# KerkDovan/univer-ocr

Measured on AMD Instinct MI355X. Metric: document-images/sec (fwd+bwd) on 256x512 synthetic pages, higher is better.
Workload: dtype f32; 1 GPU; BASELINE configs[2]: my_model train step (fwd+loss+bwd+L2+SGD) of Monochrome+Paragraph+Line on (32,256,512,1) pages and Char on (32,32,64,1) line strips per GPU; batch_per_gpu=32, global_batch=32, optimizer=sgd, parallelism=dp1, h2d_inclusive=False, input_grads=True, hip_graphs=True, pipelined_lanes=True, hw_queues=4

## Files before the change

### univer-ocr_amd/csrc/conv_fast.hip

```cpp
#include "finish_group.h"
#include "conv_dims.h"

namespace {

template <int C, typename TA>
__device__ __forceinline__ void load_vec(const TA* __restrict__ p, float (&v)[C]) {
    if constexpr (C == 1) {
        v[0] = ld1(p);
    } else if constexpr (C == 2) {
        const float2 t = ld2(p);
        v[0] = t.x;
        v[1] = t.y;
    } else {
        static_assert(C % 4 == 0, "channel count must be 1, 2 or a multiple of 4");
#pragma unroll
        for (int q = 0; q < C / 4; ++q) {
            const float4 t = ld4(p + 4 * q);
            v[4 * q] = t.x;
            v[4 * q + 1] = t.y;
            v[4 * q + 2] = t.z;
            v[4 * q + 3] = t.w;
        }
    }
}
// ... 179 lines not shown
        const bool row_ok = gy >= 0 && gy < d.oh;
        const int gyc = min(max(gy, 0), d.oh - 1);
#pragma unroll
        for (int c = 0; c < 3; ++c) {
            const int gx = i - 1 + c;
            load_vec<COUT>(gb + ((size_t)gyc * d.ow + min(max(gx, 0), d.ow - 1)) * COUT, g[r][c]);
            if (!(row_ok && gx >= 0 && gx < d.ow)) {
#pragma unroll
                for (int o = 0; o < COUT; ++o) g[r][c][o] = 0.f;
            }
        }
    }
    float out[2][2][CIN];
#pragma unroll
    for (int q = 0; q < 4; ++q)
#pragma unroll
        for (int ci = 0; ci < CIN; ++ci) out[q >> 1][q & 1][ci] = 0.f;
#pragma unroll
    for (int ky = 0; ky < 5; ++ky)
#pragma unroll
        for (int kx = 0; kx < 5; ++kx) {
            const int py = ky & 1, px = kx & 1;
            const int r = (py ? (3 - ky) / 2 : 1 - ky / 2) + 1, c = (px ? (3 - kx) / 2 : 1 - kx / 2) + 1;
#pragma unroll
            for (int ci = 0; ci < CIN; ++ci)
#pragma unroll
                for (int o = 0; o < COUT; ++o)
                    out[py][px][ci] += g[r][c][o] * w[((ky * 5 + kx) * CIN + ci) * COUT + o];
        }
#pragma unroll
    for (int py = 0; py < 2; ++py) {
        const int y = 2 * j + py;
        if (y >= d.h) break;
        const size_t off = (((size_t)b * d.h + y) * d.w + 2 * i) * CIN;
        if (CIN == 1 && (d.w & 1) == 0) {
            float v[2] = {out[py][0][0], out[py][1][0]};
            apply_mask<2>(v, mask_y, off, mask_act, mask_alpha);
            store_vec<2>(dx + off, v);
        } else {
#pragma unroll
            for (int px = 0; px < 2; ++px) {
                if (2 * i + px >= d.w) break;
                apply_mask<CIN>(out[py][px], mask_y, off + px * CIN, mask_act, mask_alpha);
                store_vec<CIN>(dx + off + px * CIN, out[py][px]);
            }
        }
    }
}

__global__ __launch_bounds__(256) void conv_dgrad_c64s2(const float* __restrict__ dy, const float* __restrict__ w,
                                                        float* __restrict__ dx, int n, int h, int wd, int oh, int ow,
                                                        const float* __restrict__ mask_y, int mask_act,
                                                        float mask_alpha) {
    constexpr int KH = 5, KW = 3, CO = 64;
    const int q = threadIdx.x & 15;
    const int b = blockIdx.z, y = blockIdx.y;
    const bool live = (int)(blockIdx.x * 16 + (threadIdx.x >> 4)) < wd;
    const int x = live ? blockIdx.x * 16 + (threadIdx.x >> 4) : wd - 1;
    const size_t pix = ((size_t)b * h + y) * wd + x;
    const float* gb = dy + (size_t)b * oh * ow * CO + 4 * q;
    float acc = 0.f;
#pragma unroll
    for (int t = 0; t < 3; ++t) {
        const int ky = (y & 1) + 2 * t, gy = (y - ky) / 2;
        if (ky >= KH || y - ky < 0 || gy >= oh) continue;
#pragma unroll
        for (int kx = 0; kx < KW; ++kx) {
            const int gx = x + 1 - kx;
            if (gx < 0 || gx >= ow) continue;
            const float4 g = *reinterpret_cast<const float4*>(gb + ((size_t)gy * ow + gx) * CO);
            const float4 wv = *reinterpret_cast<const float4*>(w + (ky * KW + kx) * CO + 4 * q);
            acc += g.x * wv.x + g.y * wv.y + g.z * wv.z + g.w * wv.w;
        }
    }
    acc += __shfl_xor(acc, 8, 64);
    acc += __shfl_xor(acc, 4, 64);
    acc += __shfl_xor(acc, 2, 64);
    acc += __shfl_xor(acc, 1, 64);
    if (!live || q != 0) return;
    if (mask_act != UOCR_ACT_NONE) acc *= act_grad_from_output<float>(mask_y[pix], mask_act, mask_alpha);
    dx[pix] = acc;
}

template <int N, int OFFS, typename TA>
__device__ __forceinline__ void load_row_c1(const TA* __restrict__ row, int a4, int width, bool row_ok,
                                            float fill, float (&seg)[N][1]) {
    constexpr int NV4 = (OFFS + N + 3) / 4;
    float buf[NV4 * 4];
#pragma unroll
    for (int k = 0; k < NV4; ++k) {
        const int col = a4 + 4 * k;
        float4 v = ld4(row + min(max(col, 0), width - 4));
        if (!(row_ok && col >= 0 && col < width)) v = make_float4(fill, fill, fill, fill);
        buf[4 * k] = v.x;
        buf[4 * k + 1] = v.y;
        buf[4 * k + 2] = v.z;
        buf[4 * k + 3] = v.w;
    }
#pragma unroll
    for (int j = 0; j < N; ++j) seg[j][0] = buf[OFFS + j];
}

template <int KH, int KW, int CIN, int COUT, int SH, int SW, int PX, typename TA, class K>
__global__ __launch_bounds__(256) void conv_fwd_px(const TA* __restrict__ x, const float* __restrict__ w,
                                                   const float* __restrict__ bias, TA* __restrict__ y,
                                                   FastDims d, float pad, int use_bias, int act, float alpha) {
    act = act_kind<K::act>(act);
    constexpr int NXV = (PX - 1) * SW + KW;
    const int ox0 = (blockIdx.x * 64 + threadIdx.x) * PX;
    const int oy = blockIdx.y * 4 + threadIdx.y;
    const int b = blockIdx.z;
    if (ox0 >= d.ow || oy >= d.oh) return;
    float acc[PX][COUT];
#pragma unroll
    for (int p = 0; p < PX; ++p)
#pragma unroll
        for (int o = 0; o < COUT; ++o) acc[p][o] = 0.f;
    const int ix0 = ox0 * SW - d.pw;
    const TA* xb = x + (size_t)b * d.h * d.w * CIN;
#pragma unroll 1
    for (int ky = 0; ky < KH; ++ky) {
        const int iy = oy * SH - d.ph + ky;
        const bool row_ok = iy >= 0 && iy < d.h;
        const TA* xr = xb + (size_t)min(max(iy, 0), d.h - 1) * d.w * CIN;
        const float* wr = w + ky * (KW * CIN * COUT);
        float xv[NXV][CIN];
        bool vec_done = false;
        if constexpr (CIN == 1 && PX % 4 == 0) {
            constexpr int PWC = KW / 2, OFFS = (4 - PWC % 4) % 4;
            if (d.pw == PWC && d.w % 4 == 0) {
                load_row_c1<NXV, OFFS>(xr, ix0 - OFFS, d.w, row_ok, pad, xv);
                vec_done = true;
            }
        }
        if (!vec_done) {
#pragma unroll
            for (int j = 0; j < NXV; ++j) {
                const int ix = ix0 + j;
                load_vec<CIN>(xr + (size_t)min(max(ix, 0), d.w - 1) * CIN, xv[j]);
                if (!(row_ok && ix >= 0 && ix < d.w)) {
#pragma unroll
                    for (int c = 0; c < CIN; ++c) xv[j][c] = pad;
                }
            }
        }
#pragma unroll
        for (int kx = 0; kx < KW; ++kx)
#pragma unroll
            for (int c = 0; c < CIN; ++c)
#pragma unroll
                for (int o = 0; o < COUT; ++o) {
                    const float wv = wr[(kx * CIN + c) * COUT + o];
#pragma unroll
                    for (int p = 0; p < PX; ++p) acc[p][o] += xv[p * SW + kx][c] * wv;
                }
    }
    if constexpr (COUT == 1 && PX % 4 == 0) {
        if (d.ow % PX == 0) {
            float out[PX];
#pragma unroll
            for (int p = 0; p < PX; ++p) out[p] = act_apply(acc[p][0] + (use_bias ? bias[0] : 0.f), act, alpha);
            store_vec<PX>(y + ((size_t)b * d.oh + oy) * d.ow + ox0, out);
            return;
        }
    }
#pragma unroll
    for (int p = 0; p < PX; ++p) {
        if (ox0 + p >= d.ow) break;
        float out[COUT];
#pragma unroll
        for (int o = 0; o < COUT; ++o) {
            float v = acc[p][o];
            if (use_bias) v += bias[o];
            out[o] = act_apply(v, act, alpha);
        }
        store_vec<COUT>(y + (((size_t)b * d.oh + oy) * d.ow + ox0 + p) * COUT, out);
    }
}

template <int KH, int KW, int CIN, int COUT, int PX, typename TA>
__global__ __launch_bounds__(256) void conv_dgrad_px(const TA* __restrict__ dy, const float* __restrict__ w,
                                                     TA* __restrict__ dx, FastDims d,
                                                     const TA* __restrict__ mask_y, int mask_act, float mask_alpha) {
    constexpr int NG = PX + KW - 1;
    const int ix0 = (blockIdx.x * 64 + threadIdx.x) * PX;
    const int iy = blockIdx.y * 4 + threadIdx.y;
    const int b = blockIdx.z;
    if (ix0 >= d.w || iy >= d.h) return;
    float acc[PX][CIN];
#pragma unroll
    for (int p = 0; p < PX; ++p)
#pragma unroll
        for (int c = 0; c < CIN; ++c) acc[p][c] = 0.f;
    const TA* gb = dy + (size_t)b * d.oh * d.ow * COUT;
    const int gx0 = ix0 + d.pw - (KW - 1);
#pragma unroll 1
    for (int ky = KH - 1; ky >= 0; --ky) {
        const int gy = iy + d.ph - ky;
        const bool row_ok = gy >= 0 && gy < d.oh;
        const TA* gr = gb + (size_t)min(max(gy, 0), d.oh - 1) * d.ow * COUT;
        const float* wr = w + ky * (KW * CIN * COUT);
        float g[NG][COUT];
        bool vec_done = false;
        if constexpr (COUT == 1 && PX % 4 == 0) {
            constexpr int PWC = KW / 2, OFFS = (((KW - 1 - PWC) % 4) + 4) % 4;
            if (d.pw == PWC && d.ow % 4 == 0) {
                load_row_c1<NG, OFFS>(gr, gx0 - OFFS, d.ow, row_ok, 0.f, g);
                vec_done = true;
            }
        }
        if (!vec_done) {
#pragma unroll
            for (int j = 0; j < NG; ++j) {
                const int gx = gx0 + j;
                load_vec<COUT>(gr + (size_t)min(max(gx, 0), d.ow - 1) * COUT, g[j]);
                if (!(row_ok && gx >= 0 && gx < d.ow)) {
#pragma unroll
                    for (int o = 0; o < COUT; ++o) g[j][o] = 0.f;
                }
            }
        }
#pragma unroll
        for (int kx = 0; kx < KW; ++kx)
#pragma unroll
            for (int c = 0; c < CIN; ++c)
#pragma unroll
                for (int o = 0; o < COUT; ++o) {
                    const float wv = wr[(kx * CIN + c) * COUT + o];
#pragma unroll
                    for (int p = 0; p < PX; ++p) acc[p][c] += g[p + (KW - 1) - kx][o] * wv;
                }
    }
    if constexpr (CIN == 1 && PX % 4 == 0) {
        if (d.w % PX == 0) {
            float out[PX];
#pragma unroll
            for (int p = 0; p < PX; ++p) out[p] = acc[p][0];
            const size_t off = ((size_t)b * d.h + iy) * d.w + ix0;
            apply_mask<PX>(out, mask_y, off, mask_act, mask_alpha);
            store_vec<PX>(dx + off, out);
            return;
        }
    }
#pragma unroll
    for (int p = 0; p < PX; ++p) {
        if (ix0 + p >= d.w) break;
        const size_t off = (((size_t)b * d.h + iy) * d.w + ix0 + p) * CIN;
        apply_mask<CIN>(acc[p], mask_y, off, mask_act, mask_alpha);
        store_vec<CIN>(dx + off, acc[p]);
    }
}

template <int KH, int KW, int PY, bool FLIP>
__global__ __launch_bounds__(256) void conv_c16_reduce(const float* __restrict__ src, const float* __restrict__ w,
                                                       const float* __restrict__ bias, float* __restrict__ dst,
                                                       int n, int h, int wd, int ph, int pw, float pad, int use_bias,
                                                       int act, float alpha, const float* __restrict__ mask_y,
                                                       int mask_act, float mask_alpha) {
    constexpr int C = 16, ROWS = PY + KH - 1;
    const int q = threadIdx.x & 3;
    const int ox = blockIdx.x * 16 + (threadIdx.x >> 2);
    const int oy0 = (blockIdx.y * 4 + threadIdx.y) * PY;
    const int b = blockIdx.z;
    float wreg[KH][KW][4];
#pragma unroll
    for (int ky = 0; ky < KH; ++ky)
#pragma unroll
        for (int kx = 0; kx < KW; ++kx) {
            const int sky = FLIP ? KH - 1 - ky : ky, skx = FLIP ? KW - 1 - kx : kx;
            const float4 t = *reinterpret_cast<const float4*>(w + (sky * KW + skx) * C + q * 4);
            wreg[ky][kx][0] = t.x;
            wreg[ky][kx][1] = t.y;
            wreg[ky][kx][2] = t.z;
            wreg[ky][kx][3] = t.w;
        }
    const int PH = FLIP ? KH - 1 - ph : ph, PW = FLIP ? KW - 1 - pw : pw;
    float acc[PY];
#pragma unroll
    for (int p = 0; p < PY; ++p) acc[p] = 0.f;
    const float* sb = src + (size_t)b * h * wd * C + q * 4;
    const int oxc = min(ox, wd - 1);
#pragma unroll
    for (int r = 0; r < ROWS; ++r) {
        const int iy = oy0 - PH + r;
        const bool row_ok = iy >= 0 && iy < h;
        const float* sr = sb + (size_t)min(max(iy, 0), h - 1) * wd * C;
#pragma unroll
        for (int kx = 0; kx < KW; ++kx) {
            const int ix = oxc - PW + kx;
            float4 v = *reinterpret_cast<const float4*>(sr + (size_t)min(max(ix, 0), wd - 1) * C);
            if (!(row_ok && ix >= 0 && ix < wd)) v = make_float4(pad, pad, pad, pad);
#pragma unroll
            for (int p = 0; p < PY; ++p) {
                const int ky = r - p;
                if (ky >= 0 && ky < KH)
                    acc[p] += v.x * wreg[ky][kx][0] + v.y * wreg[ky][kx][1] + v.z * wreg[ky][kx][2] +
                              v.w * wreg[ky][kx][3];
            }
        }
    }
#pragma unroll
    for (int p = 0; p < PY; ++p) {
        float v = acc[p];
        v += __shfl_xor(v, 1, 64);
        v += __shfl_xor(v, 2, 64);
        if (q == 0 && ox < wd && oy0 + p < h) {
            if (use_bias) v += bias[0];
            const size_t off = ((size_t)b * h + oy0 + p) * wd + ox;
            v = act_apply(v, act, alpha);
            if (mask_act != UOCR_ACT_NONE) v *= act_grad_from_output<float>(mask_y[off], mask_act, mask_alpha);
            dst[off] = v;
        }
    }
}
// ... 111 lines not shown
#pragma unroll
        for (int kx = 0; kx < KW; ++kx)
#pragma unroll
            for (int j = 0; j < 4; ++j) {
                float t = acc[ky][kx][j];
#pragma unroll
                for (int m = 4; m < 64; m <<= 1) t += __shfl_xor(t, m, 64);
                acc[ky][kx][j] = t;
            }
#pragma unroll
    for (int m = 4; m < 64; m <<= 1) accb += __shfl_xor(accb, m, 64);
    if (pl == 0) {
#pragma unroll
        for (int ky = 0; ky < KH; ++ky)
#pragma unroll
            for (int kx = 0; kx < KW; ++kx)
#pragma unroll
                for (int j = 0; j < 4; ++j) red[wv][q][(ky * KW + kx) * 4 + j] = acc[ky][kx][j];
        red[wv][q][NA - 1] = accb;
    }
    __syncthreads();
    const int tid = wv * 64 + threadIdx.x;
    float* out = partial + (size_t)blockIdx.x * 4 * NA;
    for (int a = tid; a < 4 * NA; a += 256) {
        const int qq = a / NA, i = a % NA;
        out[a] = red[0][qq][i] + red[1][qq][i] + red[2][qq][i] + red[3][qq][i];
    }
}

template <int KH, int KW>
__global__ __launch_bounds__(256) void conv_c16_wgrad_finish(const float* __restrict__ partial, float* __restrict__ dw,
                                                             float* __restrict__ db, int nblocks, int use_bias,
                                                             int accumulate) {
    constexpr int NA = KH * KW * 4 + 1;
    __shared__ double smem[16];
    const int i = blockIdx.x, q = blockIdx.y;
    double s = 0.0;
    for (int blk = threadIdx.x; blk < nblocks; blk += blockDim.x) s += (double)partial[((size_t)blk * 4 + q) * NA + i];
    s = block_reduce_sum(s, smem);
    if (threadIdx.x != 0) return;
    float* dst;
    if (i < NA - 1) {
        dst = dw + (i / 4) * 16 + q * 4 + (i % 4);
    } else {
        if (q != 0) return;
        dst = db;
        if (!use_bias) s = 0.0;
    }
    *dst = accumulate ? (float)((double)*dst + s) : (float)s;
}

template <int NP, int S>
__device__ __forceinline__ void reduce_scatter_step(float (&acc)[NP], int lane) {
    constexpr int bit = 32 >> S;
    constexpr int half = NP >> (S + 1);
    const bool up = lane & bit;
#pragma unroll
    for (int i = 0; i < half; ++i) {
        const float send = up ? acc[i] : acc[i + half];
        const float keep = up ? acc[i + half] : acc[i];
        acc[i] = keep + __shfl_xor(send, bit, 64);
    }
}

template <int NP>
__device__ __forceinline__ void lane_reduce_scatter(float (&acc)[NP], int lane) {
    reduce_scatter_step<NP, 0>(acc, lane);
    reduce_scatter_step<NP, 1>(acc, lane);
    reduce_scatter_step<NP, 2>(acc, lane);
    reduce_scatter_step<NP, 3>(acc, lane);
    reduce_scatter_step<NP, 4>(acc, lane);
    reduce_scatter_step<NP, 5>(acc, lane);
}

template <int KH, int KW, int CIN, int COUT, int SH, int SW, int KYR, int COB>
struct WgradCfg {
    static constexpr int NW = KYR * KW * CIN * COB;
    static constexpr int NACC = NW + COB;
    static constexpr int NP = ((NACC + 63) / 64) * 64;
    static constexpr int KYG = KH / KYR;
    static constexpr int OCG = COUT / COB;
};

template <int KH, int KW, int CIN, int COUT, int SH, int SW, int KYR, int COB, int PX, bool CLAMP, typename TA>
__global__ __launch_bounds__(256) void conv_wgrad_fast(const TA* __restrict__ x, const TA* __restrict__ dy,
                                                       float* __restrict__ partial, FastDims d, float pad,
                                                       int rows_per_block, int nbands) {
    using C = WgradCfg<KH, KW, CIN, COUT, SH, SW, KYR, COB>;
    constexpr int NXV = (PX - 1) * SW + KW;
    __shared__ float red[4][C::NP];
    const int lane = threadIdx.x, wv = threadIdx.y;
    const int band = blockIdx.x % nbands, b = blockIdx.x / nbands;
    const int kyg = blockIdx.y / C::OCG, ocg = blockIdx.y % C::OCG;
    const int ky0 = kyg * KYR, oc0 = ocg * COB;
    const int row0 = band * rows_per_block;
    const int row1 = min(d.oh, row0 + rows_per_block);
    float acc[C::NP];
#pragma unroll
    for (int a = 0; a < C::NP; ++a) acc[a] = 0.f;
    const TA* xb = x + (size_t)b * d.h * d.w * CIN;
    const TA* gb = dy + (size_t)b * d.oh * d.ow * COUT + oc0;
    for (int oy = row0 + wv; oy < row1; oy += 4) {
        for (int ox0 = lane * PX; ox0 < d.ow; ox0 += 64 * PX) {
            float g[PX][COB];
#pragma unroll
            for (int p = 0; p < PX; ++p) {
                if (ox0 + p < d.ow) {
                    load_vec<COB>(gb + ((size_t)oy * d.ow + ox0 + p) * COUT, g[p]);
                } else {
#pragma unroll
                    for (int o = 0; o < COB; ++o) g[p][o] = 0.f;
                }
                if (kyg == 0) {
#pragma unroll
                    for (int o = 0; o < COB; ++o) acc[C::NW + o] += g[p][o];
                }
            }
            const int iy0 = oy * SH - d.ph + ky0, ix0 = ox0 * SW - d.pw;
#pragma unroll
            for (int kyl = 0; kyl < KYR; ++kyl) {
                const int iy = iy0 + kyl;
                const bool row_ok = iy >= 0 && iy < d.h;
                const int iyc = min(max(iy, 0), d.h - 1);
                float xv[NXV][CIN];
                bool vec_done = false;
                if constexpr (CIN == 1 && PX % 4 == 0) {
                    constexpr int PWC = KW / 2, OFFS = (4 - PWC % 4) % 4;
                    if (d.pw == PWC && d.w % 4 == 0) {
                        load_row_c1<NXV, OFFS>(xb + (size_t)iyc * d.w, ix0 - OFFS, d.w, row_ok, pad, xv);
                        vec_done = true;
                    }
                }
                if (!vec_done) {
#pragma unroll
                    for (int j = 0; j < NXV; ++j) {
                        const int ix = ix0 + j;
                        if constexpr (CLAMP) {
                            load_vec<CIN>(xb + ((size_t)iyc * d.w + min(max(ix, 0), d.w - 1)) * CIN, xv[j]);
                            if (!(row_ok && ix >= 0 && ix < d.w)) {
#pragma unroll
                                for (int c = 0; c < CIN; ++c) xv[j][c] = pad;
                            }
                        } else {
                            if (row_ok && ix >= 0 && ix < d.w) {
                                load_vec<CIN>(xb + ((size_t)iy * d.w + ix) * CIN, xv[j]);
                            } else {
#pragma unroll
                                for (int c = 0; c < CIN; ++c) xv[j][c] = pad;
                            }
                        }
                    }
                }
#pragma unroll
                for (int kx = 0; kx < KW; ++kx)
#pragma unroll
                    for (int c = 0; c < CIN; ++c)
#pragma unroll
                        for (int o = 0; o < COB; ++o)
#pragma unroll
                            for (int p = 0; p < PX; ++p)
                                acc[((kyl * KW + kx) * CIN + c) * COB + o] += xv[p * SW + kx][c] * g[p][o];
            }
        }
    }
    lane_reduce_scatter<C::NP>(acc, lane);
    int base = 0;
#pragma unroll
    for (int s = 0; s < 6; ++s)
        if (lane & (32 >> s)) base += C::NP >> (s + 1);
#pragma unroll
    for (int r = 0; r < C::NP / 64; ++r) red[wv][base + r] = acc[r];
    __syncthreads();
    const int tid = wv * 64 + lane;
    float* out = partial + ((size_t)blockIdx.y * gridDim.x + blockIdx.x) * C::NP;
    for (int a = tid; a < C::NP; a += 256) out[a] = red[0][a] + red[1][a] + red[2][a] + red[3][a];
}

template <int KH, int KW, int CIN, int COUT, int KYR, int COB, int NW, int NP>
__global__ __launch_bounds__(256) void conv_wgrad_fast_finish(const float* __restrict__ partial, float* __restrict__ dw,
                                                              float* __restrict__ db, int nblocks, int use_bias,
                                                              int accumulate, float unscale) {
    __shared__ double smem[16];
    const int a = blockIdx.x, grp = blockIdx.y;
    constexpr int OCG = COUT / COB;
    const int kyg = grp / OCG, ocg = grp % OCG;
    const float* src = partial + (size_t)grp * nblocks * NP + a;
    double s = 0.0;
    for (int i = threadIdx.x; i < nblocks; i += blockDim.x) s += (double)src[(size_t)i * NP];
    s = block_reduce_sum(s, smem);
    if (threadIdx.x != 0) return;
    float* dst;
    if (a < NW) {
        const int o = a % COB, t = a / COB;
        const int c = t % CIN, tap = t / CIN;
        const int kx = tap % KW, kyl = tap / KW;
        dst = dw + (((size_t)(kyg * KYR + kyl) * KW + kx) * CIN + c) * COUT + ocg * COB + o;
    } else {
        if (kyg != 0) return;
        dst = db + ocg * COB + (a - NW);
        if (!use_bias) s = 0.0;
    }
    s *= (double)unscale;
    *dst = accumulate ? (float)((double)*dst + s) : (float)s;
}

namespace t542 {
constexpr int TH = 16, TW = 64, WH = TH + 4, WW = TW + 4, NACC = 42, NP = 64;
__device__ __forceinline__ int swz(int row, int c) { return row * WW + (c & 3) * (WW / 4) + (c >> 2); }
}

template <typename TA>
__global__ __launch_bounds__(320) void conv_wgrad_t542(const TA* __restrict__ x, const TA* __restrict__ dy,
                                                       float* __restrict__ partial, int h, int wd, float pad,
                                                       int tiles_per_block) {
    using namespace t542;
    __shared__ float4 xs[WH * WW];
    __shared__ float2 gs[TH * TW];
    const int tid = threadIdx.x, lane = tid & 63, ky = tid >> 6;
    const int x0 = blockIdx.x * TW, b = blockIdx.z;
    const int tile0 = blockIdx.y * tiles_per_block, tiles_y = (h + TH - 1) / TH;
    const TA* xb = x + (size_t)b * h * wd * 4;
    const TA* gb = dy + (size_t)b * h * wd * 2;
    float acc[NP];
#pragma unroll
    for (int a = 0; a < NP; ++a) acc[a] = 0.f;
    const int cg = lane & 15, rsub = lane >> 4;
    const int t_end = min(tiles_y, tile0 + tiles_per_block);
    for (int t = tile0; t < t_end; ++t) {
        const int y0 = t * TH;
        __syncthreads();
        for (int e = tid; e < WH * WW; e += 320) {
            const int r = e / WW, c = e - r * WW;
            const int gy = y0 - 2 + r, gx = x0 - 2 + c;
            float4 v = ld4(xb + ((size_t)min(max(gy, 0), h - 1) * wd + min(max(gx, 0), wd - 1)) * 4);
            if (gy < 0 || gy >= h || gx < 0 || gx >= wd) v = make_float4(pad, pad, pad, pad);
            xs[swz(r, c)] = v;
        }
        for (int e = tid; e < TH * TW; e += 320) {
            const int r = e / TW, c = e - r * TW;
            const int gy = y0 + r, gx = x0 + c;
            float2 v = ld2(gb + ((size_t)min(gy, h - 1) * wd + min(gx, wd - 1)) * 2);
            if (gy >= h || gx >= wd) v = make_float2(0.f, 0.f);
            gs[e] = v;
        }
        __syncthreads();
#pragma unroll 1
// ... 470 lines not shown
```

### univer-ocr_amd/csrc/conv_up.hip

```cpp
#include "up_phase.h"
#include "finish_group.h"
#include "conv_toeplitz.h"

namespace {

constexpr int CH = 4;
constexpr int RH = 16, RW = 32;
constexpr int XH = RH + 2, XW = RW + 2;
constexpr int XPLANE = 624;
constexpr int NWEFF = 9 * CH * 16;

__device__ __forceinline__ float weff_entry(const float* __restrict__ w, int i) {
    const int o = i & 3, phase = (i >> 2) & 3, c = (i >> 4) & 3, m = i >> 6;
    int ylo, yhi, xlo, xhi;
    tap_group(phase >> 1, m / 3, ylo, yhi);
    tap_group(phase & 1, m % 3, xlo, xhi);
    float v[2][2];
#pragma unroll
    for (int a = 0; a < 2; ++a)
#pragma unroll
        for (int b = 0; b < 2; ++b) v[a][b] = w[((min(ylo + a, 4) * 5 + min(xlo + b, 4)) * CH + c) * CH + o];
    float s = 0.f;
#pragma unroll
    for (int a = 0; a < 2; ++a)
// ... 340 lines not shown
    float we[36];
    weff1_build(we, w);
    const float b0 = use_bias ? bias[0] : 0.f;
    __syncthreads();
    const int c = tid & 31, r0 = tid >> 5;
    const int W = 2 * wl;
    TA* yb = y + (size_t)blockIdx.z * (2 * hl) * W;
#pragma unroll
    for (int p = 0; p < 2; ++p) {
        const int r = r0 + 8 * p, py = ry + r, pxl = rx + c;
        float acc[4] = {b0, b0, b0, b0};
#pragma unroll
        for (int m = 0; m < 9; ++m) {
            const float xv = xs[(r + m / 3) * XW + c + m % 3];
#pragma unroll
            for (int phase = 0; phase < 4; ++phase) acc[phase] += xv * we[m * 4 + phase];
        }
        if (py < hl && pxl < wl) {
            TA* o = yb + (size_t)(2 * py) * W + 2 * pxl;
            st2(o, make_float2(act_apply(acc[0], act, alpha), act_apply(acc[1], act, alpha)));
            st2(o + W, make_float2(act_apply(acc[2], act, alpha), act_apply(acc[3], act, alpha)));
        }
    }
}

template <typename TA>
__global__ __launch_bounds__(256) void up1_dgrad_kernel(const TA* __restrict__ dy, const float* __restrict__ w,
                                                        TA* __restrict__ dxl, int hl, int wl,
                                                        const TA* __restrict__ mask_y, int mask_act,
                                                        float mask_alpha) {
    __shared__ float gs[GH * GW];
    const int tid = threadIdx.x;
    const int rx = blockIdx.x * RW, ry = blockIdx.y * RH;
    const int H = 2 * hl, W = 2 * wl;
    const TA* gb = dy + (size_t)blockIdx.z * H * W;
    stage_batched<GH * GW, 256, 10, TA>(
        tid,
        [&](int i, bool& inside) {
            const int r = i / GW, c = i - r * GW;
            const int gy = 2 * (ry - 1) + r, gx = 2 * (rx - 1) + c;
            inside = gy >= 0 && gy < H && gx >= 0 && gx < W;
            return gb + (size_t)min(max(gy, 0), H - 1) * W + min(max(gx, 0), W - 1);
        },
        [&](int i, TA v, bool inside) { gs[i] = inside ? (float)v : 0.f; });
    float we[36];
    weff1_build(we, w);
    __syncthreads();
    const int c = tid & 31, r0 = tid >> 5;
#pragma unroll
    for (int p = 0; p < 2; ++p) {
        const int r = r0 + 8 * p;
        float acc = 0.f;
#pragma unroll
        for (int m = 0; m < 9; ++m) {
            const int my = m / 3 - 1, mx = m % 3 - 1;
            const float* g0 = gs + (2 * (r - my + 1)) * GW + 2 * (c - mx + 1);
            acc += we[m * 4] * g0[0] + we[m * 4 + 1] * g0[1] + we[m * 4 + 2] * g0[GW] + we[m * 4 + 3] * g0[GW + 1];
        }
        const int qy = ry + r, qx = rx + c;
        if (qy >= hl || qx >= wl) continue;
        const size_t off = ((size_t)blockIdx.z * hl + qy) * wl + qx;
        if (mask_act != UOCR_ACT_NONE) acc *= act_grad_from_output<float>(ld1(mask_y + off), mask_act, mask_alpha);
        st1(dxl + off, acc);
    }
}

template <typename TA>
__global__ __launch_bounds__(256) void up1_wgrad_kernel(const TA* __restrict__ xl, const TA* __restrict__ dy,
                                                        float* __restrict__ partial, int hl, int wl,
                                                        int rows_per_block) {
    __shared__ float xs[XH * XW];
    __shared__ float red[4][37];
    const int tid = threadIdx.x;
    const int rx = blockIdx.x * RW;
    const int row_begin = blockIdx.y * rows_per_block, row_end = min(hl, row_begin + rows_per_block);
    const TA* xb = xl + (size_t)blockIdx.z * hl * wl;
    const int W = 2 * wl;
    const TA* gb = dy + (size_t)blockIdx.z * (2 * hl) * W;
    const int c = tid & 31, r0 = tid >> 5;
    float acc[36], dbacc = 0.f;
#pragma unroll
    for (int i = 0; i < 36; ++i) acc[i] = 0.f;
    for (int ry = row_begin; ry < row_end; ry += RH) {
        __syncthreads();
        stage_batched<XH * XW, 256, 3, TA>(
            tid,
            [&](int i, bool& inside) {
                const int r = i / XW, cc = i - r * XW;
                const int gy = ry - 1 + r, gx = rx - 1 + cc;
                inside = gy >= 0 && gy < hl && gx >= 0 && gx < wl;
                return xb + (size_t)min(max(gy, 0), hl - 1) * wl + min(max(gx, 0), wl - 1);
            },
            [&](int i, TA v, bool inside) { xs[i] = inside ? (float)v : 0.f; });
        __syncthreads();
#pragma unroll
        for (int p = 0; p < 2; ++p) {
            const int r = r0 + 8 * p, py = ry + r, pxl = rx + c;
            if (py >= row_end || pxl >= wl) continue;
            const TA* g0 = gb + (size_t)(2 * py) * W + 2 * pxl;
            const float2 ga = ld2(g0), gbv = ld2(g0 + W);
            const float g[4] = {ga.x, ga.y, gbv.x, gbv.y};
            dbacc += (g[0] + g[1]) + (g[2] + g[3]);
#pragma unroll
            for (int m = 0; m < 9; ++m) {
                const float xv = xs[(r + m / 3) * XW + c + m % 3];
#pragma unroll
                for (int phase = 0; phase < 4; ++phase) acc[m * 4 + phase] += xv * g[phase];
            }
        }
    }
    const int lane = tid & 63, wv = tid >> 6;
#pragma unroll
    for (int i = 0; i < 36; ++i) {
        const float v = wave_reduce_sum(acc[i]);
        if (lane == 0) red[wv][i] = v;
    }
    dbacc = wave_reduce_sum(dbacc);
    if (lane == 0) red[wv][36] = dbacc;
    __syncthreads();
    const int blk = (blockIdx.z * gridDim.y + blockIdx.y) * gridDim.x + blockIdx.x;
    up1_write_row(partial + (size_t)blk * UP1_NOUT, [&](int i) { return red[0][i] + red[1][i] + red[2][i] + red[3][i]; }, tid);
}


int up_rows_per_block(int strips, int hl, int n, unsigned max_blocks = 2048u) {
    int rows = RH;
    while (rows < hl && (size_t)strips * ((hl + rows - 1) / rows) * n > max_blocks) rows += RH;
    return rows;
}

int check_up(uocr_ctx* ctx, int dtype, int n, int hl, int wl, int cin, int cout, int kh, int kw, int ph, int pw) {
    if (UOCR_DTYPE_BASE(dtype) != UOCR_F32 && UOCR_DTYPE_BASE(dtype) != UOCR_F16)
        UOCR_FAIL(ctx, UOCR_ERR_UNSUPPORTED, "upconv2x: float32 / float16 only");
    if (!((cin == CH && cout == CH) || (cin == 1 && cout == 1)) || kh != 5 || kw != 5 || ph != 2 || pw != 2)
        UOCR_FAIL(ctx, UOCR_ERR_UNSUPPORTED,
                  "upconv2x: 5x5 / padding 2 / 4 -> 4 or 1 -> 1 channels only (got %dx%d pad %d,%d %d -> %d)", kh, kw, ph,
                  pw, cin, cout);
    UOCR_REQUIRE(ctx, n > 0 && hl > 0 && wl > 0 && n <= 65535);
    return UOCR_OK;
}

}

extern "C" int uocr_upconv2x_fwd(uocr_ctx* ctx, int dtype, const void* x_low, const void* w, const void* b, void* y,
                                 int n, int hl, int wl, int cin, int cout, int kh, int kw, int ph, int pw,
                                 int use_bias, int act, double act_alpha, void* weff) {
    UOCR_CHECK_CTX(ctx);
    UOCR_REQUIRE(ctx, x_low && w && b && y);
    int rc = check_up(ctx, dtype, n, hl, wl, cin, cout, kh, kw, ph, pw);
    if (rc != UOCR_OK) return rc;
    if (uocr_upconv_h16_eligible(ctx, dtype, cin, cout) && uocr_aligned_act(x_low, dtype) && uocr_aligned_act(y, dtype))
        return uocr_upconv_fwd_h16(ctx, x_low, w, b, y, n, hl, wl, use_bias, act, act_alpha);
    const int strips = (wl + RW - 1) / RW, rows = up_rows_per_block(strips, hl, n, (unsigned)uocr_budget(ctx, 2048));
    if (cin != 1) uocr_note_split(ctx, (long long)strips * ((hl + rows - 1) / rows) * n, (long long)strips * ((hl + RH - 1) / RH) * n);
    return uocr_act_tags<0>(ctx, act, UOCR_ACT_NONE, [&](auto kinds) -> int {
    using K = decltype(kinds);
    UOCR_DISPATCH_TA(ctx, dtype, {
        if (cin == 1)
            hipLaunchKernelGGL((up1_fwd_kernel<TA>), dim3((wl + RW - 1) / RW, (hl + RH - 1) / RH, n), dim3(256), 0,
                               ctx->stream, (const TA*)x_low, (const float*)w, (const float*)b, (TA*)y, hl, wl, use_bias,
                               act, (float)act_alpha);
        else
            hipLaunchKernelGGL((upconv_fwd_kernel<TA, K>), dim3(strips, (hl + rows - 1) / rows, n), dim3(256), 0,
                               ctx->stream, (const TA*)x_low, (const float*)w, (const float*)b, (TA*)y, hl, wl, rows,
                               use_bias, act, (float)act_alpha, (float*)weff);
    });
    UOCR_LAUNCH_CHECK(ctx);
    return UOCR_OK;
    });
}

extern "C" int uocr_upconv2x_bwd_data(uocr_ctx* ctx, int dtype, const void* dy, const void* w, void* dx_low, int n,
                                      int hl, int wl, int cin, int cout, int kh, int kw, int ph, int pw,
                                      const void* x_act, int act, double act_alpha, const void* weff_in) {
    UOCR_CHECK_CTX(ctx);
    UOCR_REQUIRE(ctx, dy && w && dx_low);
    UOCR_REQUIRE(ctx, act == UOCR_ACT_NONE || x_act != nullptr);
    int rc = check_up(ctx, dtype, n, hl, wl, cin, cout, kh, kw, ph, pw);
    if (rc != UOCR_OK) return rc;
    if (uocr_upconv_h16_eligible(ctx, dtype, cin, cout) && uocr_aligned_act(dy, dtype) &&
        uocr_aligned_act(dx_low, dtype) && (act == UOCR_ACT_NONE || uocr_aligned_act(x_act, dtype)))
        return uocr_upconv_dgrad_h16(ctx, dy, w, dx_low, n, hl, wl, act == UOCR_ACT_NONE ? nullptr : x_act, act, act_alpha);
    if (uocr_upconv_t32_eligible(ctx, dtype, cin, cout) && uocr_aligned16(dy) && uocr_aligned16(dx_low) &&
        (act == UOCR_ACT_NONE || uocr_aligned16(x_act)))
// ... 67 lines not shown
```

Measured before the change: 34420 images/s.

## Batch and prefetch single-channel conv row loads ahead of FMA work

For single-channel stride-1 convolutions, the forward kernel now issues every kernel-row vector load up front, behind a scheduling barrier, before any FMAs. Dgrad and wgrad use a one-row-ahead software prefetch instead. Boundary handling moves to a per-row validity bitmask so the selects happen after the loads. The upsample wgrad kernel also hoists its gradient loads above the shared-memory staging barrier. The aim is to hide global-load latency, at the cost of more live VGPRs and possibly lower occupancy.

```diff
diff --git a/univer-ocr_amd/csrc/conv_fast.hip b/univer-ocr_amd/csrc/conv_fast.hip
--- a/univer-ocr_amd/csrc/conv_fast.hip
+++ b/univer-ocr_amd/csrc/conv_fast.hip
@@ -285,6 +285,35 @@
     dx[pix] = acc;
 }
 
+template <int N, int OFFS>
+struct RowC1 {
+    static constexpr int NV4 = (OFFS + N + 3) / 4;
+};
+
+template <int N, int OFFS, typename TA>
+__device__ __forceinline__ unsigned row_c1_fetch(const TA* __restrict__ row, int a4, int width,
+                                                 float4 (&v)[RowC1<N, OFFS>::NV4]) {
+    unsigned bits = 0;
+#pragma unroll
+    for (int k = 0; k < RowC1<N, OFFS>::NV4; ++k) {
+        const int col = a4 + 4 * k;
+        v[k] = ld4(row + min(max(col, 0), width - 4));
+        bits |= ((unsigned)col < (unsigned)width ? 1u : 0u) << k;
+    }
+    return bits;
+}
+
+template <int N, int OFFS>
+__device__ __forceinline__ void row_c1_select(const float4 (&v)[RowC1<N, OFFS>::NV4], unsigned bits, float fill,
+                                              float (&seg)[N][1]) {
+#pragma unroll
+    for (int j = 0; j < N; ++j) {
+        const int k = (OFFS + j) / 4, e = (OFFS + j) % 4;
+        const float t = e == 0 ? v[k].x : e == 1 ? v[k].y : e == 2 ? v[k].z : v[k].w;
+        seg[j][0] = (bits >> k) & 1u ? t : fill;
+    }
+}
+
 template <int N, int OFFS, typename TA>
 __device__ __forceinline__ void load_row_c1(const TA* __restrict__ row, int a4, int width, bool row_ok,
                                             float fill, float (&seg)[N][1]) {
@@ -302,6 +331,36 @@
     }
 #pragma unroll
     for (int j = 0; j < N; ++j) seg[j][0] = buf[OFFS + j];
+}
+
+template <int KW, int CIN, int COUT, int SW, int PX, int NXV>
+__device__ __forceinline__ void fwd_row_fma(float (&acc)[PX][COUT], const float (&xv)[NXV][CIN],
+                                            const float* __restrict__ wr) {
+#pragma unroll
+    for (int kx = 0; kx < KW; ++kx)
+#pragma unroll
+        for (int c = 0; c < CIN; ++c)
+#pragma unroll
+            for (int o = 0; o < COUT; ++o) {
+                const float wv = wr[(kx * CIN + c) * COUT + o];
+#pragma unroll
+                for (int p = 0; p < PX; ++p) acc[p][o] += xv[p * SW + kx][c] * wv;
+            }
+}
+
+template <int KW, int CIN, int COUT, int PX, int NG>
+__device__ __forceinline__ void dgrad_row_fma(float (&acc)[PX][CIN], const float (&g)[NG][COUT],
+                                              const float* __restrict__ wr) {
+#pragma unroll
+    for (int kx = 0; kx < KW; ++kx)
+#pragma unroll
+        for (int c = 0; c < CIN; ++c)
+#pragma unroll
+            for (int o = 0; o < COUT; ++o) {
+                const float wv = wr[(kx * CIN + c) * COUT + o];
+#pragma unroll
+                for (int p = 0; p < PX; ++p) acc[p][c] += g[p + (KW - 1) - kx][o] * wv;
+            }
 }
 
 template <int KH, int KW, int CIN, int COUT, int SH, int SW, int PX, typename TA, class K>
@@ -321,42 +380,59 @@
         for (int o = 0; o < COUT; ++o) acc[p][o] = 0.f;
     const int ix0 = ox0 * SW - d.pw;
     const TA* xb = x + (size_t)b * d.h * d.w * CIN;
+    constexpr bool ROW4 = CIN == 1 && PX % 4 == 0, BATCH = ROW4 && SW == 1;
+    constexpr int PWC = KW / 2, OFFS = (4 - PWC % 4) % 4;
+    bool batched = false;
+    if constexpr (BATCH) {
+        static_assert(COUT * KW <= 20, "unrolled tap rows: KH * COUT * KW weights have to fit in SGPRs");
+        if (d.pw == PWC && d.w % 4 == 0) {
+            float4 raw[KH][RowC1<NXV, OFFS>::NV4];
+            unsigned ok[KH];
+            auto fetch = [&](int ky) {
+                const int iy = oy * SH - d.ph + ky;
+                const TA* xr = xb + (size_t)min(max(iy, 0), d.h - 1) * d.w;
+                const unsigned bits = row_c1_fetch<NXV, OFFS>(xr, ix0 - OFFS, d.w, raw[ky]);
+                ok[ky] = (unsigned)iy < (unsigned)d.h ? bits : 0u;
+            };
+#pragma unroll
+            for (int ky = 0; ky < KH; ++ky) fetch(ky);
+            __builtin_amdgcn_sched_barrier(0);
+#pragma unroll
+            for (int ky = 0; ky < KH; ++ky) {
+                float xv[NXV][CIN];
+                row_c1_select<NXV, OFFS>(raw[ky], ok[ky], pad, xv);
+                fwd_row_fma<KW, CIN, COUT, SW, PX>(acc, xv, w + ky * (KW * CIN * COUT));
+            }
+            batched = true;
+        }
+    }
+    if (!batched) {
 #pragma unroll 1
-    for (int ky = 0; ky < KH; ++ky) {
-        const int iy = oy * SH - d.ph + ky;
-        const bool row_ok = iy >= 0 && iy < d.h;
-        const TA* xr = xb + (size_t)min(max(iy, 0), d.h - 1) * d.w * CIN;
-        const float* wr = w + ky * (KW * CIN * COUT);
-        float xv[NXV][CIN];
-        bool vec_done = false;
-        if constexpr (CIN == 1 && PX % 4 == 0) {
-            constexpr int PWC = KW / 2, OFFS = (4 - PWC % 4) % 4;
-            if (d.pw == PWC && d.w % 4 == 0) {
-                load_row_c1<NXV, OFFS>(xr, ix0 - OFFS, d.w, row_ok, pad, xv);
-                vec_done = true;
-            }
-        }
-        if (!vec_done) {
-#pragma unroll
-            for (int j = 0; j < NXV; ++j) {
-                const int ix = ix0 + j;
-                load_vec<CIN>(xr + (size_t)min(max(ix, 0), d.w - 1) * CIN, xv[j]);
-                if (!(row_ok && ix >= 0 && ix < d.w)) {
-#pragma unroll
-                    for (int c = 0; c < CIN; ++c) xv[j][c] = pad;
+        for (int ky = 0; ky < KH; ++ky) {
+            const int iy = oy * SH - d.ph + ky;
+            const bool row_ok = iy >= 0 && iy < d.h;
+            const TA* xr = xb + (size_t)min(max(iy, 0), d.h - 1) * d.w * CIN;
+            float xv[NXV][CIN];
+            bool vec_done = false;
+            if constexpr (ROW4 && !BATCH) {
+                if (d.pw == PWC && d.w % 4 == 0) {
+                    load_row_c1<NXV, OFFS>(xr, ix0 - OFFS, d.w, row_ok, pad, xv);
+                    vec_done = true;
                 }
             }
-        }
-#pragma unroll
-        for (int kx = 0; kx < KW; ++kx)
-#pragma unroll
-            for (int c = 0; c < CIN; ++c)
-#pragma unroll
-                for (int o = 0; o < COUT; ++o) {
-                    const float wv = wr[(kx * CIN + c) * COUT + o];
-#pragma unroll
-                    for (int p = 0; p < PX; ++p) acc[p][o] += xv[p * SW + kx][c] * wv;
+            if (!vec_done) {
+#pragma unroll
+                for (int j = 0; j < NXV; ++j) {
+                    const int ix = ix0 + j;
+                    load_vec<CIN>(xr + (size_t)min(max(ix, 0), d.w - 1) * CIN, xv[j]);
+                    if (!(row_ok && ix >= 0 && ix < d.w)) {
+#pragma unroll
+                        for (int c = 0; c < CIN; ++c) xv[j][c] = pad;
+                    }
                 }
+            }
+            fwd_row_fma<KW, CIN, COUT, SW, PX>(acc, xv, w + ky * (KW * CIN * COUT));
+        }
     }
     if constexpr (COUT == 1 && PX % 4 == 0) {
         if (d.ow % PX == 0) {
@@ -397,22 +473,43 @@
         for (int c = 0; c < CIN; ++c) acc[p][c] = 0.f;
     const TA* gb = dy + (size_t)b * d.oh * d.ow * COUT;
     const int gx0 = ix0 + d.pw - (KW - 1);
+    bool batched = false;
+    if constexpr (COUT == 1 && PX % 4 == 0) {
+        static_assert(CIN * KW <= 20, "unrolled tap rows: KH * CIN * KW weights have to fit in SGPRs");
+        constexpr int PWC = KW / 2, OFFS = (((KW - 1 - PWC) % 4) + 4) % 4;
+        constexpr int AHEAD = 1;
+        if (d.pw == PWC && d.ow % 4 == 0) {
+            float4 raw[KH][RowC1<NG, OFFS>::NV4];
+            unsigned ok[KH];
+            auto fetch = [&](int t) {
+                const int gy = iy + d.ph - (KH - 1 - t);
+                const TA* gr = gb + (size_t)min(max(gy, 0), d.oh - 1) * d.ow;
+                const unsigned bits = row_c1_fetch<NG, OFFS>(gr, gx0 - OFFS, d.ow, raw[t]);
+                ok[t] = (unsigned)gy < (unsigned)d.oh ? bits : 0u;
+            };
+#pragma unroll
+            for (int t = 0; t < AHEAD; ++t) fetch(t);
+            __builtin_amdgcn_sched_barrier(0);
+#pragma unroll
+            for (int t = 0; t < KH; ++t) {
+                if (t + AHEAD < KH) {
+                    fetch(t + AHEAD);
+                    __builtin_amdgcn_sched_barrier(0);
+                }
+                float g[NG][COUT];
+                row_c1_select<NG, OFFS>(raw[t], ok[t], 0.f, g);
+                dgrad_row_fma<KW, CIN, COUT, PX>(acc, g, w + (KH - 1 - t) * (KW * CIN * COUT));
+            }
+            batched = true;
+        }
+    }
+    if (!batched) {
 #pragma unroll 1
-    for (int ky = KH - 1; ky >= 0; --ky) {
-        const int gy = iy + d.ph - ky;
-        const bool row_ok = gy >= 0 && gy < d.oh;
-        const TA* gr = gb + (size_t)min(max(gy, 0), d.oh - 1) * d.ow * COUT;
-        const float* wr = w + ky * (KW * CIN * COUT);
-        float g[NG][COUT];
-        bool vec_done = false;
-        if constexpr (COUT == 1 && PX % 4 == 0) {
-            constexpr int PWC = KW / 2, OFFS = (((KW - 1 - PWC) % 4) + 4) % 4;
-            if (d.pw == PWC && d.ow % 4 == 0) {
-                load_row_c1<NG, OFFS>(gr, gx0 - OFFS, d.ow, row_ok, 0.f, g);
-                vec_done = true;
-            }
-        }
-        if (!vec_done) {
+        for (int ky = KH - 1; ky >= 0; --ky) {
+            const int gy = iy + d.ph - ky;
+            const bool row_ok = gy >= 0 && gy < d.oh;
+            const TA* gr = gb + (size_t)min(max(gy, 0), d.oh - 1) * d.ow * COUT;
+            float g[NG][COUT];
 #pragma unroll
             for (int j = 0; j < NG; ++j) {
                 const int gx = gx0 + j;
@@ -422,17 +519,8 @@
                     for (int o = 0; o < COUT; ++o) g[j][o] = 0.f;
                 }
             }
-        }
-#pragma unroll
-        for (int kx = 0; kx < KW; ++kx)
-#pragma unroll
-            for (int c = 0; c < CIN; ++c)
-#pragma unroll
-                for (int o = 0; o < COUT; ++o) {
-                    const float wv = wr[(kx * CIN + c) * COUT + o];
-#pragma unroll
-                    for (int p = 0; p < PX; ++p) acc[p][c] += g[p + (KW - 1) - kx][o] * wv;
-                }
+            dgrad_row_fma<KW, CIN, COUT, PX>(acc, g, w + ky * (KW * CIN * COUT));
+        }
     }
     if constexpr (CIN == 1 && PX % 4 == 0) {
         if (d.w % PX == 0) {
@@ -710,6 +798,54 @@
     static constexpr int OCG = COUT / COB;
 };
 
+template <int KW, int SH, int SW, int KYR, int PX, int NW, int NP, typename TA>
+__device__ __forceinline__ void wgrad_step_c1(float (&acc)[NP], const TA* __restrict__ xb, const TA* __restrict__ gb,
+                                              const FastDims& d, float pad, int oy, int ox0, int ky0, bool with_db) {
+    constexpr int NXV = (PX - 1) * SW + KW, PWC = KW / 2, OFFS = (4 - PWC % 4) % 4;
+    constexpr int AHEAD = 1;
+    const int iy0 = oy * SH - d.ph + ky0, ix0 = ox0 * SW - d.pw;
+    float4 gv[PX / 4];
+#pragma unroll
+    for (int q = 0; q < PX / 4; ++q) gv[q] = ld4(gb + (size_t)oy * d.ow + min(ox0 + 4 * q, d.ow - 4));
+    float4 raw[KYR][RowC1<NXV, OFFS>::NV4];
+    unsigned ok[KYR];
+    auto fetch = [&](int kyl) {
+        const int iy = iy0 + kyl;
+        const TA* xr = xb + (size_t)min(max(iy, 0), d.h - 1) * d.w;
+        const unsigned bits = row_c1_fetch<NXV, OFFS>(xr, ix0 - OFFS, d.w, raw[kyl]);
+        ok[kyl] = (unsigned)iy < (unsigned)d.h ? bits : 0u;
+    };
+#pragma unroll
+    for (int kyl = 0; kyl < AHEAD; ++kyl) fetch(kyl);
+    __builtin_amdgcn_sched_barrier(0);
+    float g[PX];
+#pragma unroll
+    for (int q = 0; q < PX / 4; ++q) {
+        const bool in = ox0 + 4 * q < d.ow;
+        g[4 * q] = in ? gv[q].x : 0.f;
+        g[4 * q + 1] = in ? gv[q].y : 0.f;
+        g[4 * q + 2] = in ? gv[q].z : 0.f;
+        g[4 * q + 3] = in ? gv[q].w : 0.f;
+    }
+    if (with_db) {
+#pragma unroll
+        for (int p = 0; p < PX; ++p) acc[NW] += g[p];
+    }
+#pragma unroll
+    for (int kyl = 0; kyl < KYR; ++kyl) {
+        if (kyl + AHEAD < KYR) {
+            fetch(kyl + AHEAD);
+            __builtin_amdgcn_sched_barrier(0);
+        }
+        float xv[NXV][1];
+        row_c1_select<NXV, OFFS>(raw[kyl], ok[kyl], pad, xv);
+#pragma unroll
+        for (int kx = 0; kx < KW; ++kx)
+#pragma unroll
+            for (int p = 0; p < PX; ++p) acc[kyl * KW + kx] += xv[p * SW + kx][0] * g[p];
+    }
+}
+
 template <int KH, int KW, int CIN, int COUT, int SH, int SW, int KYR, int COB, int PX, bool CLAMP, typename TA>
 __global__ __launch_bounds__(256) void conv_wgrad_fast(const TA* __restrict__ x, const TA* __restrict__ dy,
                                                        float* __restrict__ partial, FastDims d, float pad,
@@ -728,68 +864,69 @@
     for (int a = 0; a < C::NP; ++a) acc[a] = 0.f;
     const TA* xb = x + (size_t)b * d.h * d.w * CIN;
     const TA* gb = dy + (size_t)b * d.oh * d.ow * COUT + oc0;
-    for (int oy = row0 + wv; oy < row1; oy += 4) {
-        for (int ox0 = lane * PX; ox0 < d.ow; ox0 += 64 * PX) {
-            float g[PX][COB];
-#pragma unroll
-            for (int p = 0; p < PX; ++p) {
-                if (ox0 + p < d.ow) {
-                    load_vec<COB>(gb + ((size_t)oy * d.ow + ox0 + p) * COUT, g[p]);
+    auto step = [&](int oy, int ox0) {
+        float g[PX][COB];
+#pragma unroll
+        for (int p = 0; p < PX; ++p) {
+            if (ox0 + p < d.ow) {
+                load_vec<COB>(gb + ((size_t)oy * d.ow + ox0 + p) * COUT, g[p]);
+            } else {
+#pragma unroll
+                for (int o = 0; o < COB; ++o) g[p][o] = 0.f;
+            }
+            if (kyg == 0) {
+#pragma unroll
+                for (int o = 0; o < COB; ++o) acc[C::NW + o] += g[p][o];
+            }
+        }
+        const int iy0 = oy * SH - d.ph + ky0, ix0 = ox0 * SW - d.pw;
+#pragma unroll
+        for (int kyl = 0; kyl < KYR; ++kyl) {
+            const int iy = iy0 + kyl;
+            const bool row_ok = iy >= 0 && iy < d.h;
+            const int iyc = min(max(iy, 0), d.h - 1);
+            float xv[NXV][CIN];
+#pragma unroll
+            for (int j = 0; j < NXV; ++j) {
+                const int ix = ix0 + j;
+                if constexpr (CLAMP) {
+                    load_vec<CIN>(xb + ((size_t)iyc * d.w + min(max(ix, 0), d.w - 1)) * CIN, xv[j]);
+                    if (!(row_ok && ix >= 0 && ix < d.w)) {
+#pragma unroll
+                        for (int c = 0; c < CIN; ++c) xv[j][c] = pad;
+                    }
                 } else {
-#pragma unroll
-                    for (int o = 0; o < COB; ++o) g[p][o] = 0.f;
-                }
-                if (kyg == 0) {
-#pragma unroll
-                    for (int o = 0; o < COB; ++o) acc[C::NW + o] += g[p][o];
-                }
-            }
-            const int iy0 = oy * SH - d.ph + ky0, ix0 = ox0 * SW - d.pw;
-#pragma unroll
-            for (int kyl = 0; kyl < KYR; ++kyl) {
-                const int iy = iy0 + kyl;
-                const bool row_ok = iy >= 0 && iy < d.h;
-                const int iyc = min(max(iy, 0), d.h - 1);
-                float xv[NXV][CIN];
-                bool vec_done = false;
-                if constexpr (CIN == 1 && PX % 4 == 0) {
-                    constexpr int PWC = KW / 2, OFFS = (4 - PWC % 4) % 4;
-                    if (d.pw == PWC && d.w % 4 == 0) {
-                        load_row_c1<NXV, OFFS>(xb + (size_t)iyc * d.w, ix0 - OFFS, d.w, row_ok, pad, xv);
-                        vec_done = true;
+                    if (row_ok && ix >= 0 && ix < d.w) {
+                        load_vec<CIN>(xb + ((size_t)iy * d.w + ix) * CIN, xv[j]);
+                    } else {
+#pragma unroll
+                        for (int c = 0; c < CIN; ++c) xv[j][c] = pad;
                     }
                 }
-                if (!vec_done) {
-#pragma unroll
-                    for (int j = 0; j < NXV; ++j) {
-                        const int ix = ix0 + j;
-                        if constexpr (CLAMP) {
-                            load_vec<CIN>(xb + ((size_t)iyc * d.w + min(max(ix, 0), d.w - 1)) * CIN, xv[j]);
-                            if (!(row_ok && ix >= 0 && ix < d.w)) {
-#pragma unroll
-                                for (int c = 0; c < CIN; ++c) xv[j][c] = pad;
-                            }
-                        } else {
-                            if (row_ok && ix >= 0 && ix < d.w) {
-                                load_vec<CIN>(xb + ((size_t)iy * d.w + ix) * CIN, xv[j]);
-                            } else {
-#pragma unroll
-                                for (int c = 0; c < CIN; ++c) xv[j][c] = pad;
-                            }
-                        }
-                    }
-                }
-#pragma unroll
-                for (int kx = 0; kx < KW; ++kx)
-#pragma unroll
-                    for (int c = 0; c < CIN; ++c)
-#pragma unroll
-                        for (int o = 0; o < COB; ++o)
-#pragma unroll
-                            for (int p = 0; p < PX; ++p)
-                                acc[((kyl * KW + kx) * CIN + c) * COB + o] += xv[p * SW + kx][c] * g[p][o];
-            }
-        }
+            }
+#pragma unroll
+            for (int kx = 0; kx < KW; ++kx)
+#pragma unroll
+                for (int c = 0; c < CIN; ++c)
+#pragma unroll
+                    for (int o = 0; o < COB; ++o)
+#pragma unroll
+                        for (int p = 0; p < PX; ++p)
+                            acc[((kyl * KW + kx) * CIN + c) * COB + o] += xv[p * SW + kx][c] * g[p][o];
+        }
+    };
+    bool vec_done = false;
+    if constexpr (CIN == 1 && COUT == 1 && PX % 4 == 0) {
+        if (d.pw == KW / 2 && d.w % 4 == 0 && d.ow % 4 == 0) {
+            for (int oy = row0 + wv; oy < row1; oy += 4)
+                for (int ox0 = lane * PX; ox0 < d.ow; ox0 += 64 * PX)
+                    wgrad_step_c1<KW, SH, SW, KYR, PX, C::NW>(acc, xb, gb, d, pad, oy, ox0, ky0, kyg == 0);
+            vec_done = true;
+        }
+    }
+    if (!vec_done) {
+        for (int oy = row0 + wv; oy < row1; oy += 4)
+            for (int ox0 = lane * PX; ox0 < d.ow; ox0 += 64 * PX) step(oy, ox0);
     }
     lane_reduce_scatter<C::NP>(acc, lane);
     int base = 0;
diff --git a/univer-ocr_amd/csrc/conv_up.hip b/univer-ocr_amd/csrc/conv_up.hip
--- a/univer-ocr_amd/csrc/conv_up.hip
+++ b/univer-ocr_amd/csrc/conv_up.hip
@@ -446,6 +446,13 @@
 #pragma unroll
     for (int i = 0; i < 36; ++i) acc[i] = 0.f;
     for (int ry = row_begin; ry < row_end; ry += RH) {
+        float2 gv[2][2];
+#pragma unroll
+        for (int p = 0; p < 2; ++p) {
+            const TA* g0 = gb + (size_t)(2 * min(ry + r0 + 8 * p, hl - 1)) * W + 2 * min(rx + c, wl - 1);
+            gv[p][0] = ld2(g0);
+            gv[p][1] = ld2(g0 + W);
+        }
         __syncthreads();
         stage_batched<XH * XW, 256, 3, TA>(
             tid,
@@ -461,9 +468,7 @@
         for (int p = 0; p < 2; ++p) {
             const int r = r0 + 8 * p, py = ry + r, pxl = rx + c;
             if (py >= row_end || pxl >= wl) continue;
-            const TA* g0 = gb + (size_t)(2 * py) * W + 2 * pxl;
-            const float2 ga = ld2(g0), gbv = ld2(g0 + W);
-            const float g[4] = {ga.x, ga.y, gbv.x, gbv.y};
+            const float g[4] = {gv[p][0].x, gv[p][0].y, gv[p][1].x, gv[p][1].y};
             dbacc += (g[0] + g[1]) + (g[2] + g[3]);
 #pragma unroll
             for (int m = 0; m < 9; ++m) {
```

After: 34580 images/s (median of 6 runs). Within noise of the previous version (+0.5%).
